# jackbaggins/RayTracing2-fork

Measured on AMD Instinct MI355X. Metric: Msamples/sec at 1920×1080 Cornell+OBJ; per-pixel RMSE vs CPU ref, higher is better.
Workload: dtype f32

## Files before the change

### raytracing2-fork_amd/csrc/device/rt2_k5_resident.h

```cpp
#pragma once

extern "C" __device__ int rt2_writelane(int value, int lane, int old) __asm("llvm.amdgcn.writelane.i32");

namespace {

constexpr int kResGroups = 38;

struct K5Resident {
    h8 rec[kResGroups * 4 * 64];
};

template <MfmaSpec S>
__device__ __forceinline__ bool exact_group(unsigned long long M, int G, int n_tris, cfloat* tri, const f3& o,
                                            const f3& d, float& best, int& bi, float& bestK, MfmaDiag& dg) {
    if constexpr (S.diag) dg.hot += 1;
    uint32_t m32 = (uint32_t)(M | M >> 32);
    const float bk0 = bestK;
    while (m32) {
        const int tt = __builtin_ctz(m32);
        m32 &= m32 - 1;
        const int idx = 32 * G + tt;
        if (idx >= n_tris) break;
        if constexpr (S.diag) dg.exact += 1;
        cfloat* tp = tri + 12 * idx;
        const MtQ qq = mt_quantities(o, d, ldc4(tp), ldc4(tp + 4), ldc4(tp + 8));
        if (mt_pass3(qq, bestK)) mt_exact(qq, idx, best, bi, bestK);
    }
    return __ballot(bestK != bk0) != 0;
}

__device__ __forceinline__ void xl_counts(MfmaDiag& dg, int pairs, int k, int rounds) {
    for (int off = 32; off > 0; off >>= 1) {
        pairs += __shfl_xor(pairs, off);
        k = max(k, __shfl_xor(k, off));
    }
    const unsigned long long kw = (unsigned long long)__builtin_amdgcn_readfirstlane(k);
    dg.xl[0] += (unsigned long long)__builtin_amdgcn_readfirstlane(pairs);
    dg.xl[1] += kw;
    dg.xl[2] += (unsigned long long)rounds;
    dg.xl[3] = kw > dg.xl[3] ? kw : dg.xl[3];
}

__host__ __device__ constexpr int xl_row_of_bit(int b) { return 8 * ((b & 15) >> 2) + 4 * (b >> 4) + (b & 3); }
__host__ __device__ constexpr int xl_bit_of_row(int r) { return 16 * ((r >> 2) & 1) + 4 * (r >> 3) + (r & 3); }

template <MfmaSpec S, bool YP, bool LDS, class Rebuild>
__device__ __forceinline__ void exact_window_lanes(int maskv, int Gw, bool more, int n_tris, const float4* tri4,
                                                   const h8* a0, const h8* y1, const h8* recs, bool upper, const f3& o,
                                                   const f3& d, float& best, int& bi, float& bestK, MfmaDiag& dg,
                                                   Rebuild rebuild, [[maybe_unused]] const int* slot_tri = nullptr) {
    const int lane = (int)lane_id();
    [[maybe_unused]] unsigned long long tc = 0;
    if constexpr (S.diag) {
        dg.claims += 1;
        tc = __builtin_amdgcn_s_memtime();
    }
    if (n_tris & 31) maskv = lane == (n_tris >> 5) - Gw ? maskv & (int)((1u << (n_tris & 31)) - 1u) : maskv;
    unsigned long long hotg = __ballot(maskv != 0);
    if constexpr (S.diag) dg.hot += (unsigned long long)__popcll(hotg);
    const float bk0 = bestK;
    const int src = 4 * xl_bit_of_row(lane & 31);
    const f16v zero = {};
    uint32_t m = 0;
    int gj = 0;
    [[maybe_unused]] int pairs = 0, iters = 0, rounds = 0;
#pragma nounroll
    for (;;) {
        int lst = 0, c = 0;
#pragma nounroll
        while (c < 32) {
            if (!m) {
                if (!hotg) break;
                gj = __builtin_ctzll(hotg);
                hotg &= hotg - 1;
                m = (uint32_t)__builtin_amdgcn_readlane(maskv, gj);
            }
            const int idx = 32 * (Gw + gj) + __builtin_ctz(m);
            m &= m - 1;
            lst = lane == c ? idx : lst;
            c++;
        }
        if (!c) break;
        if constexpr (S.diag) {
            dg.exact += (unsigned long long)c;
// ... 29 lines not shown
        };
        const int mk0 = block(0);
        int mk1 = 0;
        if (upper) mk1 = block(1);
        const auto sw = __builtin_amdgcn_permlane32_swap((uint32_t)mk0, (uint32_t)mk1, false, false);
        uint32_t pm = (sw[0] | sw[1] << 16) & (c == 32 ? ~0u : (1u << c) - 1u);
        if constexpr (S.diag) pairs += __popc(pm);
        auto entry = [&](uint32_t m) { return __builtin_amdgcn_ds_bpermute(4 * __builtin_ctz(m | 0x80000000u), lst); };
        struct Tri {
            int idx;
            float4 t0, t1, t2;
        };
        auto fetch = [&](Tri& t) {
            t.idx = entry(pm);
            t.t0 = tri4[3 * t.idx], t.t1 = tri4[3 * t.idx + 1], t.t2 = tri4[3 * t.idx + 2];
        };
        auto step = [&](const Tri& cur, Tri& nxt) {
            if constexpr (S.diag) iters += 1;
            const bool has = pm != 0;
            pm &= pm - 1;
            fetch(nxt);
            if (has) {
                const MtQ qq = mt_quantities(o, d, cur.t0, cur.t1, cur.t2);
                if (mt_pass3(qq, bestK)) {
                    if constexpr (S.slot_order)
                        mt_exact_slot(qq, cur.idx, slot_tri, best, bi, bestK);
                    else
                        mt_exact(qq, cur.idx, best, bi, bestK);
                }
            }
        };
        Tri ta, tb2;
        fetch(ta);
#pragma nounroll
        while (__ballot(pm != 0)) {
            step(ta, tb2);
            if (!__ballot(pm != 0)) break;
            step(tb2, ta);
        }
        if (c < 32) break;
    }
    if constexpr (S.diag) xl_counts(dg, pairs, iters, rounds);
    if (more && __ballot(bestK != bk0)) {
        if constexpr (S.diag) tc = __builtin_amdgcn_s_memtime();
        rebuild();
        if constexpr (S.diag) dg.t_pub += __builtin_amdgcn_s_memtime() - tc;
    }
}

template <MfmaSpec S, class Rebuild>
__device__ __forceinline__ void exact_window(uint32_t m1, int maskv, int Gw, int cnt, bool more, int n_tris,
                                             cfloat* tri, const f3& o, const f3& d, float& best, int& bi,
                                             float& bestK, MfmaDiag& dg, Rebuild rebuild) {
    constexpr int W = S.exact_win;
    auto mask_of = [&](int j) { return W == 1 ? m1 : (uint32_t)__builtin_amdgcn_readlane(maskv, j); };
    [[maybe_unused]] unsigned long long tc = 0;
    if constexpr (S.diag) {
        dg.claims += 1;
        tc = __builtin_amdgcn_s_memtime();
        int j = 0;
        while (!mask_of(j)) j++;
        const int idx = 32 * (Gw + j) + __builtin_ctz(mask_of(j));
        if (idx < n_tris) asm volatile("" ::"s"(__float_as_int(tri[12 * idx])));
        const unsigned long long t = __builtin_amdgcn_s_memtime();
        dg.t_issue += t - tc;
    }
    const float bk0 = bestK;
    [[maybe_unused]] int pairs = 0, tested = 0;
    for (int j = 0; j < cnt; j++) {
        uint32_t m32 = mask_of(j);
        if constexpr (S.diag) dg.hot += m32 != 0;
// ... 102 lines not shown
    const uint32_t dst = row + (row & 16);
    const auto sw = __builtin_amdgcn_permlane32_swap(dst, dst, false, false);
    const int half = (l & 32) >> 1;
    const int to0 = 4 * ((int)sw[0] + half), to1 = 4 * ((int)sw[1] + half);
    const u4 b0 = __builtin_bit_cast(u4, a0[0]), b1 = __builtin_bit_cast(u4, a0[1]);
    const bool first = (l & 15) < c0, keep = (l & 0x28) == 0;
    u4 r;
#pragma unroll
    for (int k = 0; k < 4; k++) {
        const int x0 = __builtin_amdgcn_ds_permute(to0, (int)b0[k]);
        const int x1 = __builtin_amdgcn_ds_permute(to1, (int)b1[k]);
        const uint32_t q = (uint32_t)(first ? x0 : x1);
        const uint32_t up = __builtin_amdgcn_permlane32_swap(0u, q, false, false)[0];
        const uint32_t sh = (uint32_t)__builtin_amdgcn_update_dpp(0, (int)up, 0x118, 0xf, 0xf, true);
        r[k] = keep ? q : sh;
    }
    return __builtin_bit_cast(h8, r);
}

struct SlotImage {
    const float4* tri4;
    const int* slot_tri;
};
__device__ __forceinline__ SlotImage slot_image(const RenderParams& p) {
    const int ng = (p.n_tris + 31) >> 5;
    const char* tab = reinterpret_cast<const char*>(reinterpret_cast<const h8*>(p.mfma_kt_frag) + (size_t)ng * (kKtOps * 64));
    const float4* t4 = reinterpret_cast<const float4*>(tab + sizeof(rt2_cluster_table));
    return {t4, reinterpret_cast<const int*>(t4 + 3 * (size_t)p.n_tris)};
}

template <MfmaSpec S>
__device__ __forceinline__ bool sweep_kt_res(const RenderParams& p, const h8* rec, const f3& o, const f3& d,
                                             float& best, int& bi, float& bestK, MfmaDiag& dg, bool upper,
                                             unsigned long long act = 0, ClusterDiag* cd = nullptr) {
    const int lane = (int)lane_id();
    [[maybe_unused]] unsigned long long tc = 0, tsw = 0;
    if constexpr (S.diag) tsw = tc = __builtin_amdgcn_s_memtime();
    auto stamp = [&](unsigned long long& acc) {
        if constexpr (S.diag) {
            const unsigned long long t = __builtin_amdgcn_s_memtime();
            acc += t - tc;
            tc = t;
        }
    };
    const f3 m = cross(d, o);
    MfmaScale sc;
    if (!mfma_scale<true>(p.mfma_A, o, d, m, sc)) return false;
    h8 a0[2], y1[2];
    _Float16 tw16;
    kt_frags<S.kt_lane_w>(d, m, sc, a0, tw16);
    constexpr bool per_group = S.exact_win == 1 && !S.y_skip_last && !S.diag;
    if constexpr (per_group || S.y_first) kt_y(d, o, bestK, sc, tw16, y1);
    stamp(dg.t_wait);
    const int ng = (p.n_tris + 31) >> 5, n_tris = p.n_tris;
    const int nres = S.res_l2 ? min(ng, kResGroups) : ng;
    cfloat* const tri = (cfloat*)p.tri;
    const h8* tb = rec + lane;
    [[maybe_unused]] const int* slot_tri = nullptr;
    if constexpr (S.slot_order) {
        static_assert(S.cluster_rows && S.exact_lanes && !S.res_l2, "slot_order: 353 / 354's one resident window");
        slot_tri = slot_image(p).slot_tri;
    }
    if constexpr (per_group) {
        for (int G = 0; G < nres; G++) {
            const h8 b0 = tb[0], b1 = tb[64], b2 = tb[128], b3 = tb[192];
            tb += kKtOps * 64;
            const unsigned long long M = kt_group(a0, y1, b0, b1, b2, b3, upper);
// ... 182 lines not shown
                            } else {
                                h8 af = a0[0];
                                if (upper) af = cluster_rows_frag(a0, need);
                                one_block(af, g0, g1);
                            }
                        }
                        maskv = lane < kNeedLane ? maskv : 0;
                    }
                }
            } else {
                for (int j = 0; j < cnt; j++) {
                    const h8 b0 = tb[0], b1 = tb[64], b2 = tb[128];
                    h8 b3 = {};
                    if constexpr (YP) b3 = tb[192];
                    tb += kKtOps * 64;
                    const unsigned long long M = kt_group<YP>(a0, y1, b0, b1, b2, b3, upper);
                    const uint32_t m32 = (uint32_t)(M | M >> 32);
                    if constexpr (W > 1) maskv = lane == j ? (int)m32 : maskv;
                    any |= m32;
                }
            }
            if constexpr (S.diag) dg.groups += (unsigned long long)cnt;
            if (resident) stamp(dg.t_filt);
            if (any) {
                const bool more = YP && (Gw + cnt < ng || (W == 1 && !S.y_skip_last));
                if (resident) phase_prio<S>(1);
                if constexpr (S.exact_lanes) {
                    static_assert(W > 1, "exact_lanes reads the window's masks from maskv");
                    const float4* tri4 = reinterpret_cast<const float4*>(p.tri);
                    if constexpr (S.slot_order) tri4 = slot_image(p).tri4;
                    auto rebuild = [&] { kt_y(d, o, bestK, sc, tw16, y1); };
                    if (!YP || resident)
                        exact_window_lanes<S, YP, true>(maskv, Gw, more, n_tris, tri4, a0, y1, rec, upper, o, d, best,
                                                        bi, bestK, dg, rebuild, slot_tri);
                    else if constexpr (YP)
                        exact_window_lanes<S, YP, false>(maskv, Gw, more, n_tris, tri4, a0, y1,
                                                         reinterpret_cast<const h8*>(p.mfma_kt_frag), upper, o, d, best,
                                                         bi, bestK, dg, rebuild);
                } else {
                    exact_window<S>(any, maskv, Gw, cnt, more, n_tris, tri, o, d, best, bi, bestK, dg,
                                    [&] { kt_y(d, o, bestK, sc, tw16, y1); });
                }
                if (resident) phase_prio<S>(0);
            }
            if constexpr (!YP && (S.res_l2 || W < kResGroups))
                if (Gw + cnt < ng) {
                    [[maybe_unused]] unsigned long long ty = 0;
                    if constexpr (S.diag) ty = __builtin_amdgcn_s_memtime();
                    kt_y(d, o, bestK, sc, tw16, y1);
                    if constexpr (S.diag) dg.t_pub += __builtin_amdgcn_s_memtime() - ty;
                }
            if (resident) stamp(dg.t_exact);
        };
        auto windows = [&](auto yfirst, const h8* tb, int G0, int G1, bool resident) {
            constexpr bool YF = decltype(yfirst)::value;
            int Gw = G0;
            if constexpr (!YF) {
                if (Gw < G1) window(std::false_type{}, tb, Gw, G1, resident);
                Gw += W;
            }
            if constexpr (YF || W < kResGroups)
                for (; Gw < G1; Gw += W) window(std::true_type{}, tb, Gw, G1, resident);
        };
        windows(std::bool_constant<S.y_first>{}, tb, 0, nres, true);
        if constexpr (S.res_l2)
            windows(std::true_type{}, reinterpret_cast<const h8*>(p.mfma_kt_frag) + (size_t)nres * (kKtOps * 64) + lane,
                    nres, ng, false);
// ... 16 lines not shown
        const h8* src = reinterpret_cast<const h8*>(p.mfma_kt_frag) + (size_t)pc * 64 + lane;
        __builtin_amdgcn_global_load_lds((const __attribute__((address_space(1))) void*)src,
                                         (__attribute__((address_space(3))) void*)&rs.rec[pc * 64], 16, 0, 0);
    }
    asm volatile("s_waitcnt vmcnt(0)" ::: "memory");
    __syncthreads();
}

template <MfmaSpec S>
__global__ __launch_bounds__(S.block) __attribute__((amdgpu_waves_per_eu(S.waves))) void render_mfma_k5r(RenderParams p_arg) {
    constexpr int NW = S.block / 64;
    __shared__ K5Resident rs;
    {
        const RenderParams& p = kargs<RenderParams>();
        const int ng = min((p.n_tris + 31) >> 5, kResGroups);
        const int lane = (int)lane_id(), wave = (int)(threadIdx.x >> 6);
        constexpr bool no_t1 = !S.y_first && S.exact_win >= kResGroups && !S.res_l2;
        for (int i = wave; i < (no_t1 ? 3 : 4) * ng; i += NW) {
            const int pc = no_t1 ? i + i / 3 : i;
            const h8* src = reinterpret_cast<const h8*>(p.mfma_kt_frag) + (size_t)pc * 64 + lane;
            __builtin_amdgcn_global_load_lds((const __attribute__((address_space(1))) void*)src,
                                             (__attribute__((address_space(3))) void*)&rs.rec[pc * 64], 16, 0, 0);
        }
        asm volatile("s_waitcnt vmcnt(0)" ::: "memory");
        __syncthreads();
    }
    Lane L;
    lane_init(L);
    MfmaDiag dg;
    struct NoClusterDiag {};
    [[maybe_unused]] std::conditional_t<S.cluster_rows8, ClusterDiag8,
                                        std::conditional_t<S.cluster_rows, ClusterDiag, NoClusterDiag>> cdg;
    [[maybe_unused]] PathDiagSlot<S.diag> pds;
    const int wave = (int)(threadIdx.x >> 6);
    [[maybe_unused]] unsigned long long segs_w = 0;
    [[maybe_unused]] unsigned long long wl_t0 = 0, wl_c0 = 0, wl_dry = 0, wl_r2 = 0, wl_r1 = 0, wl_coop = 0;
    if constexpr (S.diag) {
        wl_t0 = __builtin_amdgcn_s_memrealtime();
        wl_c0 = __builtin_amdgcn_s_memtime();
    }
    for (;;) {
        const RenderParams& p = kargs<RenderParams>();
        if constexpr (S.cam_park) {
            constexpr bool no_t1 = !S.y_first && S.exact_win >= kResGroups && !S.res_l2;
            static_assert(no_t1 && S.lean && NW <= kResGroups, "cam_park parks in T1 pieces that nothing else uses");
            float4* park = reinterpret_cast<float4*>(&rs.rec[(4 * wave + 3) * 64 + (int)lane_id()]);
            if constexpr (S.diag)
                advance<1, false, true, true, S.linear>(L, p, park, pds.get());
            else
                advance<1, false, true, false, S.linear>(L, p, park);
        } else if constexpr (S.diag) {
            advance<1, !S.lean, false, true, S.linear>(L, p, nullptr, pds.get());
        } else {
            advance<1, !S.lean, false, false, S.linear>(L, p);
        }
        unsigned long long act = __ballot(L.st == ST_TRACE);
        if constexpr (S.lean) segs_w += (unsigned long long)__popcll(act);
        if constexpr (S.diag) {
            if (!wl_dry && __any(L.st == ST_DONE)) wl_dry = __builtin_amdgcn_s_memrealtime();
            if (act) {
                if (__popcll(act) <= (unsigned)S.tail_lanes && __any(L.st == ST_DONE))
                    wl_coop++;
                else if (__popcll(act) <= 32)
                    wl_r1++;
                else
                    wl_r2++;
            }
// ... 26 lines not shown
                __builtin_amdgcn_s_setprio(0);
        }
        bool upper = true;
        if (__popcll(act) <= 32) {
            if (act >> 32) {
                const uint32_t l = lane_id(), nl = (uint32_t)__popcll(act);
                const bool live = (act >> l) & 1ull;
                const int to = 4 * (int)(live ? lanes_below(act) : nl + lanes_below(~act));
                lane_permute<!S.lean, !S.lean>(L, to);
                if constexpr (S.cam_park) {
                    float4* park = reinterpret_cast<float4*>(&rs.rec[(4 * wave + 3) * 64 + (int)lane_id()]);
                    const float4 e = *park;
                    *park = make_float4(perm_f(to, e.x), perm_f(to, e.y), perm_f(to, e.z), 0.0f);
                }
                act = __ballot(L.st == ST_TRACE);
            }
            upper = false;
        }
        const int j0 = __builtin_ctzll(act);
        const bool mine = L.st == ST_TRACE;
        {
            const f3 o = mk(__shfl(L.o.x, j0), __shfl(L.o.y, j0), __shfl(L.o.z, j0));
            const f3 dd = mk(__shfl(L.d.x, j0), __shfl(L.d.y, j0), __shfl(L.d.z, j0));
            if (!mine) {
                L.o = o;
                L.d = dd;
            }
        }
        const f3 ro = L.o, rd = L.d;
        float best = 1e38f, bestK = 1e38f * 1.0009765625f;
        int bi = -1;
        phase_prio<S>(0);
        bool swept;
        if constexpr (S.cluster_rows)
            swept = sweep_kt_res<S>(p, rs.rec, ro, rd, best, bi, bestK, dg, upper, act, &cdg);
        else
            swept = sweep_kt_res<S>(p, rs.rec, ro, rd, best, bi, bestK, dg, upper);
        if (!swept) coop_each(act, ro, rd, p, best, bi);
        phase_prio<S>(2);
        if (mine) {
            L.bounce += 1;
            if constexpr (!S.lean) L.segs += 1;
            if constexpr (S.diag)
                shade<1, true, S.linear>(L, p, best, bi, pds.get());
            else
                shade<1, false, S.linear>(L, p, best, bi);
        }
    }
    const RenderParams& p = kargs<RenderParams>();
    if constexpr (S.lean) {
        if (lane_id() == 0) atomicAdd(p.seg_counter, segs_w);
    } else {
        flush_counters(L, p);
    }
    if constexpr (S.diag)
        if (p.wave_log) {
            const uint32_t gw = blockIdx.x * NW + (uint32_t)wave;
            const unsigned long long c1 = __builtin_amdgcn_s_memtime();
            const unsigned long long hw = (unsigned long long)__builtin_amdgcn_s_getreg((31 << 11) | 4) |
                                          (unsigned long long)__builtin_amdgcn_s_getreg((15 << 11) | 20) << 32;
            if (lane_id() == 0 && gw < p.wave_log_n) {
                unsigned long long* e = p.wave_log + 10 * (size_t)gw;
                e[0] = wl_t0;
                e[1] = wl_dry;
                e[2] = __builtin_amdgcn_s_memrealtime();
                e[3] = wl_r2;
                e[4] = wl_r1;
// ... 12 lines not shown
        }
        if (lane_id() == 0) {
            atomicAdd(p.seg_counter + 20, calls);
            atomicAdd(p.seg_counter + 21, trips);
        }
    }
    if constexpr (S.diag)
        if (lane_id() == 0) {
            atomicAdd(p.seg_counter + 1, dg.groups);
            atomicAdd(p.seg_counter + 2, dg.hot);
            atomicAdd(p.seg_counter + 3, dg.exact);
            atomicAdd(p.seg_counter + 12, dg.t_wait);
            atomicAdd(p.seg_counter + 13, dg.t_filt);
            atomicAdd(p.seg_counter + 14, dg.t_exact);
            atomicAdd(p.seg_counter + 15, dg.t_swp);
            atomicAdd(p.seg_counter + 16, __builtin_amdgcn_s_memtime() - wl_c0);
            atomicAdd(p.seg_counter + 17, dg.t_issue);
            atomicAdd(p.seg_counter + 18, dg.t_pub);
            atomicAdd(p.seg_counter + 19, dg.claims);
            atomicAdd(p.seg_counter + 7, dg.xl[0]);
            atomicAdd(p.seg_counter + 8, dg.xl[1]);
            atomicAdd(p.seg_counter + 9, dg.xl[2]);
            atomicMax(p.seg_counter + 10, dg.xl[3]);
            atomicAdd(p.seg_counter + 22, pds.d.new_ray);
            atomicAdd(p.seg_counter + 23, pds.d.new_px);
            if constexpr (S.cluster_rows) {
                atomicAdd(p.seg_counter + 24, cdg.skipped);
                atomicAdd(p.seg_counter + 25, cdg.one);
                atomicAdd(p.seg_counter + 26, cdg.two);
                atomicAdd(p.seg_counter + 27, cdg.rays);
                atomicAdd(p.seg_counter + 28, cdg.r16);
                if constexpr (S.cluster_rows8) atomicAdd(p.seg_counter + 30, cdg.r8);
            }
        }
}

}
```

### raytracing2-fork_amd/csrc/device/rt2_mfma.h

```cpp
#pragma once

namespace {

typedef _Float16 h8 __attribute__((ext_vector_type(8)));
typedef float f4v __attribute__((ext_vector_type(4)));
typedef float f16v __attribute__((ext_vector_type(16)));

constexpr int kMfmaQ = 5;
constexpr float kMfmaC = 1.0009765625f;
constexpr float kMfmaTs = 0x1p-12f;
constexpr float kMfmaB = 2.0f;

struct MfmaSpec {
    int block;
    int waves;
    int tail_lanes;
    bool diag = false;
    int tile_groups = 0;
    bool fair_prio = false;
    int phase_prio = 0;
    bool flow_prio = false;
    bool kt_lane_w = false;
    bool lean = false;
    bool res_l2 = false;
    int exact_win = 1;
    bool y_skip_last = false;
    bool y_first = false;
    bool exact_lanes = false;
    bool pair_loop = false;
    bool cam_park = false;
    bool cluster_rows = false;
    bool cluster_rows16 = false;
    bool cluster_rows8 = false;
    bool slot_order = false;
    bool linear = false;
};

struct MfmaDiag {
    unsigned long long groups = 0, hot = 0, exact = 0;
    unsigned long long xl[4] = {};
    unsigned long long t_wait = 0, t_filt = 0, t_exact = 0, t_swp = 0;
    unsigned long long unused1 = 0;
    unsigned long long t_issue = 0, t_pub = 0, claims = 0;
};

struct MfmaCoef {
    double c[kMfmaQ][10];
    double tau;
};
__device__ __forceinline__ void mfma_coefs(const float4* tri, int i, int n, MfmaCoef& k, uint32_t* flags) {
    for (int q = 0; q < kMfmaQ; q++)
        for (int c = 0; c < 10; c++) k.c[q][c] = 0.0;
    k.tau = 1.0;
    if (i >= n) {
        k.c[3][9] = 0x1p13;
        return;
    }
    const float4 t0 = tri[3 * i], t1 = tri[3 * i + 1], t2 = tri[3 * i + 2];
    const float a[3] = {t0.x, t0.y, t0.z}, e0[3] = {t0.w, t1.x, t1.y}, e1[3] = {t1.z, t1.w, t2.x},
                nn[3] = {t2.y, t2.z, t2.w};
    bool ok = true;
    float A = 0.0f, M = 0.0f;
    for (int j = 0; j < 3; j++) {
        ok = ok && fabsf(a[j]) <= 0x1p20f;
        A = fmaxf(A, fabsf(a[j]));
        for (float x : {e0[j], e1[j], nn[j]}) {
            const float ax = fabsf(x);
            ok = ok && (x == 0.0f || (ax >= 0x1p-100f && ax <= 0x1p20f));
// ... 1001 lines not shown
```

### raytracing2-fork_amd/csrc/device/rt2_render.hip

```cpp
#include <hip/hip_runtime.h>

#include <algorithm>
#include <cstdio>
#include <cstdlib>
#include <cstring>
#include <mutex>
#include <numeric>
#include <string>
#include <type_traits>
#include <vector>

#include "../../../include/rt2.h"
#include "../../../include/rt2_cluster.h"
#include "rt2_math.h"

using namespace rt2d;

#include "rt2_sweep.h"
#include "rt2_path.h"
#include "rt2_brute.h"
#include "rt2_mfma.h"
#include "rt2_k5_tiles.h"
#include "rt2_k5_resident.h"
#include "rt2_assist.h"
// ... 557 lines not shown
    x.y_first = true;
    return x;
}
#endif
constexpr MfmaSpec kt_xl(MfmaSpec x) {
    x.exact_lanes = true;
    return x;
}
constexpr MfmaSpec kt_pair(MfmaSpec x) {
    x.pair_loop = true;
    return x;
}
constexpr MfmaSpec kt_park(MfmaSpec x) {
    x.cam_park = true;
    return x;
}
constexpr MfmaSpec kt_cr(MfmaSpec x) {
    x.cluster_rows = true;
    return x;
}
constexpr MfmaSpec kt_cr16(MfmaSpec x) {
    x.cluster_rows = true;
    x.cluster_rows16 = true;
    return x;
}
constexpr MfmaSpec kt_cr8(MfmaSpec x) {
    x.cluster_rows8 = true;
    return x;
}
constexpr MfmaSpec kt_slot(MfmaSpec x) {
    x.slot_order = true;
    return x;
}
constexpr int kResWin = 38;
constexpr int kResL2Groups = 256;
constexpr MfmaSpec kt_tiles_flow() {
    return MfmaSpec{.block = 768, .waves = 3, .tail_lanes = 0, .tile_groups = 19, .flow_prio = true, .kt_lane_w = true};
}
constexpr MfmaSpec kt_tiles_flow4() {
    MfmaSpec x = kt_tiles_flow();
    x.block = 1024;
    x.waves = 4;
    x.lean = true;
    return x;
}
constexpr MfmaSpec kResFrame = kt_win(kt_res(false, false, true, 4), kResWin);
constexpr MfmaSpec kResSlabFrame = kt_win(kt_res(false, true, true), kResWin);
constexpr MfmaSpec kt_product(MfmaSpec frame) { return kt_slot(kt_cr8(kt_cr16(kt_park(kt_pair(kt_xl(frame)))))); }
constexpr MfmaSpec kRes = kt_product(kResFrame);
constexpr MfmaSpec kResSlab = kt_product(kResSlabFrame);
constexpr MfmaSpec kResL2 = kt_win(kt_res(true, false, true, 4), kResWin);
constexpr MfmaSpec kResL2Slab = kt_win(kt_res(true, true, true), kResWin);
constexpr MfmaSpec kTiles = kt_tiles_flow4();
constexpr Bvh3Spec kBvhDefault{.block = 256, .thresh = 16, .slab = Slab::Markstein, .waves = 5, .diag = false};

#ifdef RT2_EXPERIMENTS
constexpr SmemSpec smem_x(int g, Filter f, Tail t, int lanes, int w, bool stats = false) {
    return SmemSpec{.block = 256, .group = g, .filter = f, .tail = t, .tail_lanes = lanes, .waves = w, .stats = stats};
}
constexpr SplitSpec split_x(int s, Filter f, int w) {
    return SplitSpec{.waves_per_ray = s, .group = 8, .filter = f, .waves = w};
}
constexpr Bvh3Spec bvh3_x(int t, Slab sl, int w, bool diag = false) {
    return Bvh3Spec{.block = 256, .thresh = t, .slab = sl, .waves = w, .diag = diag};
}
#endif

constexpr Variant kVariants[] = {
    RT2_VARIANT(0, K_SMEM, render_smem<kSmemDefault>, 256, "smem/256/max3f8/coop32/w6/lockstep"),
    RT2_PRODUCT(109, K_BVH4, render_bvh4, kBvhDefault, 256, "bvh4/256/t16/w5"),
    RT2_PRODUCT(86, K_TILED, render_tiled, kTiledLarge, 512, "tiled/512/max3f4"),
    RT2_PRODUCT(92, K_ASSIST, render_assist, kAssist12, 768, "assist12/max3f8/w6"),
    RT2_PRODUCT(136, K_SMEM, render_smem, kSmemDefault, 256, "smem/256/max3f8/coop32/w6/lockstep"),
    RT2_PRODUCT(227, K_MFMA, render_mfma, kMfmaK5, 256, "mfma/256/k5/coop8/w3/imax/minred/ymma/t12/llds/ser4/cmp"),
    RT2_PRODUCT(353, K_MFMA, render_mfma_k5r, kRes, 1024, "mfmar/1024/kt4/res38/coop4/w4/cmp/dpp/lean/lw/pp4", kResGroups, true),
    RT2_PRODUCT(354, K_MFMA, render_mfma_k5r, kResSlab, 1024, "mfmar/1024/kt4/res38/coop4/w4/cmp/fair/dpp/lean/lw", kResGroups, true),
    RT2_PRODUCT(355, K_MFMA, render_mfma_k5r, kResL2, 1024, "mfmarl2/1024/kt4/res38l2/coop4/w4/cmp/dpp/lean/lw/pp4", kResL2Groups),
    RT2_PRODUCT(356, K_MFMA, render_mfma_k5r, kResL2Slab, 1024, "mfmarl2/1024/kt4/res38l2/coop4/w4/cmp/fair/dpp/lean/lw", kResL2Groups),
    RT2_PRODUCT(380, K_MFMA, render_mfma_k5t, kTiles, 1024, "mfmat5/1024/kt4/tile19/coop0/w4/cmp/regs/perm/lw/flowp/lean"),
#ifdef RT2_EXPERIMENTS
    RT2_VARIANT(342, K_MFMA, render_mfma_k5r<kt_win(kt_res(false, false, false), kResWin)>, 1024, "mfmar/1024/kt4/res38/coop4/w4/cmp/dpp/lean", kResGroups),
// ... 7 lines not shown
    RT2_VARIANT(350, K_MFMA, render_mfma_k5r<kt_win(kt_res(false, false, true, 0, true), kResWin)>, 1024, "mfmar/1024/kt4/res38/coop4/w4/cmp/diag/dpp/lean/lw", kResGroups),
    RT2_VARIANT(390, K_MFMA, render_mfma_k5r<kt_win(kt_res(false, false, true, 0, true), 1)>, 1024, "mfmar/1024/kt4/res38/coop4/w4/cmp/diag/dpp/lean/lw/xw1", kResGroups),
    RT2_VARIANT(392, K_MFMA, render_mfma_k5r<kt_win(kt_res(false, false, true, 4), 1)>, 1024, "mfmar/1024/kt4/res38/coop4/w4/cmp/dpp/lean/lw/pp4/xw1", kResGroups),
    RT2_VARIANT(393, K_MFMA, render_mfma_k5r<kt_win(kt_res(false, false, true, 4), 1, true)>, 1024, "mfmar/1024/kt4/res38/coop4/w4/cmp/dpp/lean/lw/pp4/xw1s", kResGroups),
    RT2_VARIANT(394, K_MFMA, render_mfma_k5r<kt_win(kt_res(false, false, true, 4), 2)>, 1024, "mfmar/1024/kt4/res38/coop4/w4/cmp/dpp/lean/lw/pp4/xw2", kResGroups),
    RT2_VARIANT(395, K_MFMA, render_mfma_k5r<kt_win(kt_res(false, false, true, 4), 4)>, 1024, "mfmar/1024/kt4/res38/coop4/w4/cmp/dpp/lean/lw/pp4/xw4", kResGroups),
    RT2_VARIANT(396, K_MFMA, render_mfma_k5r<kt_win(kt_res(false, false, true, 4), 8)>, 1024, "mfmar/1024/kt4/res38/coop4/w4/cmp/dpp/lean/lw/pp4/xw8", kResGroups),
    RT2_VARIANT(399, K_MFMA, render_mfma_k5r<kt_win(kt_res(false, false, true, 4), 19)>, 1024, "mfmar/1024/kt4/res38/coop4/w4/cmp/dpp/lean/lw/pp4/xw19", kResGroups),
    RT2_VARIANT(397, K_MFMA, render_mfma_k5r<kt_win(kt_res(true, false, true, 4), 1)>, 1024, "mfmarl2/1024/kt4/res38l2/coop4/w4/cmp/dpp/lean/lw/pp4/xw1", kResL2Groups),
    RT2_VARIANT(398, K_MFMA, render_mfma_k5r<kt_win(kt_res(false, true, true), 1)>, 1024, "mfmar/1024/kt4/res38/coop4/w4/cmp/fair/dpp/lean/lw/xw1", kResGroups),
    RT2_VARIANT(351, K_MFMA, render_mfma_k5r<kt_yw(kt_win(kt_res(false, false, true, 4), kResWin))>, 1024, "mfmar/1024/kt4/res38/coop4/w4/cmp/dpp/lean/lw/pp4/yw", kResGroups),
    RT2_VARIANT(352, K_MFMA, render_mfma_k5r<kt_yw(kt_win(kt_res(true, false, true, 4), kResWin))>, 1024, "mfmarl2/1024/kt4/res38l2/coop4/w4/cmp/dpp/lean/lw/pp4/yw", kResL2Groups),
    RT2_VARIANT(357, K_MFMA, render_mfma_k5r<kt_yw(kt_win(kt_res(false, false, true, 0, true), kResWin))>, 1024, "mfmar/1024/kt4/res38/coop4/w4/cmp/diag/dpp/lean/lw/yw", kResGroups),
    RT2_VARIANT(400, K_MFMA, render_mfma_k5r<kt_win(kt_res(false, false, true, 4), kResWin)>, 1024, "mfmar/1024/kt4/res38/coop4/w4/cmp/dpp/lean/lw/pp4/xwave", kResGroups),
    RT2_VARIANT(401, K_MFMA, render_mfma_k5r<kt_xl(kt_win(kt_res(true, false, true, 4), kResWin))>, 1024, "mfmarl2/1024/kt4/res38l2/coop4/w4/cmp/dpp/lean/lw/pp4/xl", kResL2Groups),
    RT2_VARIANT(402, K_MFMA, render_mfma_k5r<kt_xl(kt_win(kt_res(false, false, true, 0, true), kResWin))>, 1024, "mfmar/1024/kt4/res38/coop4/w4/cmp/diag/dpp/lean/lw/xl", kResGroups),
    RT2_VARIANT(403, K_MFMA, render_mfma_k5r<kt_win(kt_res(false, true, true), kResWin)>, 1024, "mfmar/1024/kt4/res38/coop4/w4/cmp/fair/dpp/lean/lw/xwave", kResGroups),
    RT2_VARIANT(404, K_MFMA, render_mfma_k5r<kt_xl(kt_win(kt_res(true, true, true), kResWin))>, 1024, "mfmarl2/1024/kt4/res38l2/coop4/w4/cmp/fair/dpp/lean/lw/xl", kResL2Groups),
    RT2_VARIANT(405, K_MFMA, render_mfma_k5r<kt_xl(kt_win(kt_res(false, false, true, 4), kResWin))>, 1024, "mfmar/1024/kt4/res38/coop4/w4/cmp/dpp/lean/lw/pp4/nopair/nopark", kResGroups),
    RT2_VARIANT(406, K_MFMA, render_mfma_k5r<kt_pair(kt_xl(kt_win(kt_res(false, false, true, 4), kResWin)))>, 1024, "mfmar/1024/kt4/res38/coop4/w4/cmp/dpp/lean/lw/pp4/nopark", kResGroups),
    RT2_VARIANT(407, K_MFMA, render_mfma_k5r<kt_park(kt_xl(kt_win(kt_res(false, false, true, 4), kResWin)))>, 1024, "mfmar/1024/kt4/res38/coop4/w4/cmp/dpp/lean/lw/pp4/nopair", kResGroups),
    RT2_VARIANT(408, K_MFMA, render_mfma_k5r<kt_xl(kt_win(kt_res(false, true, true), kResWin))>, 1024, "mfmar/1024/kt4/res38/coop4/w4/cmp/fair/dpp/lean/lw/nopair/nopark", kResGroups),
    RT2_VARIANT(409, K_MFMA, render_mfma_k5r<kt_park(kt_pair(kt_xl(kt_win(kt_res(false, false, true, 4), kResWin))))>, 1024, "mfmar/1024/kt4/res38/coop4/w4/cmp/dpp/lean/lw/pp4/nocr", kResGroups),
    RT2_VARIANT(410, K_MFMA, render_mfma_k5r<kt_park(kt_pair(kt_xl(kt_win(kt_res(false, true, true), kResWin))))>, 1024, "mfmar/1024/kt4/res38/coop4/w4/cmp/fair/dpp/lean/lw/nocr", kResGroups),
    RT2_VARIANT(411, K_MFMA, render_mfma_k5r<kt_cr16(kt_pair(kt_xl(kt_win(kt_res(false, false, true, 0, true), kResWin))))>, 1024, "mfmar/1024/kt4/res38/coop4/w4/cmp/diag/dpp/lean/lw/xl/cr16", kResGroups),
    RT2_VARIANT(412, K_MFMA, render_mfma_k5r<kt_cr(kt_park(kt_pair(kt_xl(kt_win(kt_res(false, false, true, 4), kResWin)))))>, 1024, "mfmar/1024/kt4/res38/coop4/w4/cmp/dpp/lean/lw/pp4/cr32", kResGroups),
    RT2_VARIANT(413, K_MFMA, render_mfma_k5r<kt_cr(kt_park(kt_pair(kt_xl(kt_win(kt_res(false, true, true), kResWin)))))>, 1024, "mfmar/1024/kt4/res38/coop4/w4/cmp/fair/dpp/lean/lw/cr32", kResGroups),
    RT2_VARIANT(414, K_MFMA, render_mfma_k5r<kt_cr16(kt_park(kt_pair(kt_xl(kt_win(kt_res(false, false, true, 4), kResWin)))))>, 1024, "mfmar/1024/kt4/res38/coop4/w4/cmp/dpp/lean/lw/pp4/idx", kResGroups),
    RT2_VARIANT(415, K_MFMA, render_mfma_k5r<kt_cr16(kt_park(kt_pair(kt_xl(kt_win(kt_res(false, true, true), kResWin)))))>, 1024, "mfmar/1024/kt4/res38/coop4/w4/cmp/fair/dpp/lean/lw/idx", kResGroups),
    RT2_VARIANT(416, K_MFMA, render_mfma_k5r<kt_slot(kt_cr16(kt_pair(kt_xl(kt_win(kt_res(false, false, true, 0, true), kResWin)))))>, 1024, "mfmar/1024/kt4/res38/coop4/w4/cmp/diag/dpp/lean/lw/xl/cr16/slot", kResGroups, true),
    RT2_VARIANT(417, K_MFMA, render_mfma_k5r<kt_slot(kt_cr16(kt_park(kt_pair(kt_xl(kt_win(kt_res(false, false, true, 4), kResWin))))))>, 1024, "mfmar/1024/kt4/res38/coop4/w4/cmp/dpp/lean/lw/pp4/r16", kResGroups, true),
    RT2_VARIANT(418, K_MFMA, render_mfma_k5r<kt_slot(kt_cr16(kt_park(kt_pair(kt_xl(kt_win(kt_res(false, true, true), kResWin))))))>, 1024, "mfmar/1024/kt4/res38/coop4/w4/cmp/fair/dpp/lean/lw/r16", kResGroups, true),
    RT2_VARIANT(419, K_MFMA, render_mfma_k5r<kt_slot(kt_cr8(kt_cr16(kt_pair(kt_xl(kt_win(kt_res(false, false, true, 0, true), kResWin))))))>, 1024, "mfmar/1024/kt4/res38/coop4/w4/cmp/diag/dpp/lean/lw/xl/cr8/slot", kResGroups, true),
    RT2_VARIANT(370, K_MFMA, render_mfma_k5t<kt_tiles_flow()>, 768, "mfmat5/768/kt4/tile19/coop0/w3/cmp/regs/perm/lw/flowp"),
    RT2_VARIANT(368, K_MFMA, render_mfma_k5t<[] { MfmaSpec x = kt_tiles_flow(); x.diag = true; return x; }()>, 768, "mfmat5/768/kt4/tile19/coop0/w3/cmp/regs/perm/lw/flowp/diag"),
    RT2_VARIANT(369, K_MFMA, render_mfma_k5t<[] { MfmaSpec x = kt_tiles_flow(); x.flow_prio = false; return x; }()>, 768, "mfmat5/768/kt4/tile19/coop0/w3/cmp/regs/perm/lw/flow"),
    RT2_VARIANT(382, K_MFMA, render_mfma_k5t<[] { MfmaSpec x = kt_tiles_flow(); x.lean = true; return x; }()>, 768, "mfmat5/768/kt4/tile19/coop0/w3/cmp/regs/perm/lw/flowp/lean"),
    RT2_VARIANT(381, K_MFMA, render_mfma_k5t<[] { MfmaSpec x = kt_tiles_flow4(); x.tile_groups = 16; return x; }()>, 1024, "mfmat5/1024/kt4/tile16/coop0/w4/cmp/regs/perm/lw/flowp/lean"),
    RT2_VARIANT(385, K_MFMA, render_mfma_k5t<[] { MfmaSpec x = kt_tiles_flow4(); x.flow_prio = false; return x; }()>, 1024, "mfmat5/1024/kt4/tile19/coop0/w4/cmp/regs/perm/lw/flow/lean"),
    RT2_VARIANT(386, K_MFMA, render_mfma_k5t<[] { MfmaSpec x = kt_tiles_flow4(); x.tail_lanes = 4; return x; }()>, 1024, "mfmat5/1024/kt4/tile19/coop4/w4/cmp/regs/perm/lw/flowp/lean"),
    RT2_VARIANT(67, K_SMEM, render_smem<kSmemMid>, 256, "smem/256/max3f8/coop32"),
    RT2_VARIANT(85, K_SPLIT, render_split<kSplitSmall>, 256, "split4/max3f8/w6"),
    RT2_VARIANT(53, K_BVH3, render_bvh3<kBvhDefault>, 256, "bvh3/256/t16/w5"),
    RT2_VARIANT(106, K_SMEM, render_smem<kSmemFree>, 256, "smem/256/max3f8/coop32/w6/free"),
    RT2_VARIANT(37, K_BVH, render_bvh<BvhSpec{256}>, 256, "bvh/256"),
    RT2_VARIANT(40, K_BVH2, (render_bvh2<Bvh2Spec{256, 16}>), 256, "bvh2/256/t16"),
    RT2_VARIANT(41, K_BVH2, (render_bvh2<Bvh2Spec{256, 8}>), 256, "bvh2/256/t8"),
    RT2_VARIANT(43, K_BVH2, (render_bvh2<Bvh2Spec{128, 16}>), 128, "bvh2/128/t16"),
    RT2_VARIANT(45, K_BVH2, (render_bvh2<Bvh2Spec{256, 1}>), 256, "bvh2/256/t1"),
    RT2_VARIANT(46, K_BVH3, render_bvh3<bvh3_x(16, Slab::Markstein, 1)>, 256, "bvh3/256/t16"),
    RT2_VARIANT(47, K_BVH3, render_bvh3<bvh3_x(8, Slab::Markstein, 1)>, 256, "bvh3/256/t8"),
    RT2_VARIANT(48, K_BVH3, render_bvh3<bvh3_x(24, Slab::Markstein, 1)>, 256, "bvh3/256/t24"),
    RT2_VARIANT(50, K_BVH3, render_bvh3<bvh3_x(16, Slab::Binary64, 1)>, 256, "bvh3/256/t16/div64"),
    RT2_VARIANT(54, K_BVH3, render_bvh3<bvh3_x(8, Slab::Markstein, 5)>, 256, "bvh3/256/t8/w5"),
    RT2_VARIANT(55, K_BVH3, render_bvh3<bvh3_x(16, Slab::Filtered, 5)>, 256, "bvh3/256/t16/filt/w5"),
    RT2_VARIANT(58, K_BVH3, render_bvh3<bvh3_x(16, Slab::Markstein, 5, true)>, 256, "bvh3/256/t16/w5/DIAG"),
    RT2_VARIANT(64, K_SMEM, render_smem<smem_x(8, Filter::Five, Tail::Team, 32, 1)>, 256, "smem/256/masked8/team32"),
    RT2_VARIANT(66, K_SMEM, render_smem<smem_x(8, Filter::Five, Tail::Team, 64, 1)>, 256, "smem/256/masked8/team64"),
    RT2_VARIANT(74, K_SMEM, render_smem<smem_x(4, Filter::Plk, Tail::Coop, 32, 1)>, 256, "smem/256/plk4/coop32"),
    RT2_VARIANT(76, K_SMEM, render_smem<smem_x(8, Filter::Plk, Tail::Coop, 32, 1)>, 256, "smem/256/plk8/coop32"),
    RT2_VARIANT(79, K_SMEM, render_smem<smem_x(8, Filter::Plk, Tail::Coop, 32, 6)>, 256, "smem/256/plk8/coop32/w6"),
    RT2_VARIANT(80, K_SMEM, render_smem<smem_x(2, Filter::Plk, Tail::Coop, 32, 1)>, 256, "smem/256/plk2/coop32"),
    RT2_VARIANT(82, K_SMEM, render_smem<smem_x(8, Filter::Max3, Tail::Coop, 32, 1, true)>, 256,
                "smem/256/max3f8/coop32/STATS"),
#endif
};
// ... 1225 lines not shown
```

Measured before the change: 2011.

## Spread leftover exact triangle tests across idle lanes via LDS work list

After each lane handles its first candidate triangle in the exact window, the remaining (lane, triangle) pairs are prefix-summed with a DPP scan and written to an LDS list. When they fit in one wave pass, each lane takes one pair, pulls that ray's origin, direction and best hit with ds_bpermute, and runs the exact Möller–Trumbore test. Results merge back through a wave-scoped 64-bit atomic min per ray slot. This replaces the divergent serial loop over remaining hits, at the cost of LDS traffic, permutes and atomics, and it becomes the default in kt_product.

```diff
diff --git a/raytracing2-fork_amd/csrc/device/rt2_k5_resident.h b/raytracing2-fork_amd/csrc/device/rt2_k5_resident.h
--- a/raytracing2-fork_amd/csrc/device/rt2_k5_resident.h
+++ b/raytracing2-fork_amd/csrc/device/rt2_k5_resident.h
@@ -44,12 +44,37 @@
 __host__ __device__ constexpr int xl_row_of_bit(int b) { return 8 * ((b & 15) >> 2) + 4 * (b >> 4) + (b & 3); }
 __host__ __device__ constexpr int xl_bit_of_row(int r) { return 16 * ((r >> 2) & 1) + 4 * (r >> 3) + (r & 3); }
 
+template <int CTRL, int ROW_MASK>
+__device__ __forceinline__ int dpp_add_step(int x) {
+    return x + __builtin_amdgcn_update_dpp(0, x, CTRL, ROW_MASK, 0xf, false);
+}
+__device__ __forceinline__ int exact_spread_scan(int r, int& at) {
+    int x = r;
+    x = dpp_add_step<0x111, 0xf>(x);
+    x = dpp_add_step<0x112, 0xf>(x);
+    x = dpp_add_step<0x114, 0xf>(x);
+    x = dpp_add_step<0x118, 0xf>(x);
+    x = dpp_add_step<0x142, 0xa>(x);
+    x = dpp_add_step<0x143, 0xc>(x);
+    at = x - r;
+    return __builtin_amdgcn_readlane(x, 63);
+}
+
 template <MfmaSpec S, bool YP, bool LDS, class Rebuild>
 __device__ __forceinline__ void exact_window_lanes(int maskv, int Gw, bool more, int n_tris, const float4* tri4,
                                                    const h8* a0, const h8* y1, const h8* recs, bool upper, const f3& o,
                                                    const f3& d, float& best, int& bi, float& bestK, MfmaDiag& dg,
-                                                   Rebuild rebuild, [[maybe_unused]] const int* slot_tri = nullptr) {
+                                                   Rebuild rebuild, [[maybe_unused]] const int* slot_tri = nullptr,
+                                                   [[maybe_unused]] unsigned long long* xs_diag = nullptr,
+                                                   [[maybe_unused]] int xs_wave = 0) {
     const int lane = (int)lane_id();
+    [[maybe_unused]] uint32_t* xs_list = nullptr;
+    [[maybe_unused]] unsigned long long* xs_slot = nullptr;
+    constexpr bool XS = S.exact_spread && LDS && !YP;
+    if constexpr (XS) {
+        xs_list = reinterpret_cast<uint32_t*>(const_cast<h8*>(recs) + (4 * (16 + xs_wave) + 3) * 64);
+        xs_slot = reinterpret_cast<unsigned long long*>(xs_list + 128);
+    }
     [[maybe_unused]] unsigned long long tc = 0;
     if constexpr (S.diag) {
         dg.claims += 1;
@@ -145,11 +170,95 @@
         };
         Tri ta, tb2;
         fetch(ta);
+        if constexpr (XS) {
+            {
+                if constexpr (S.diag) iters += 1;
+                const bool has = pm != 0;
+                pm &= pm - 1;
+                if (has) {
+                    const MtQ qq = mt_quantities(o, d, ta.t0, ta.t1, ta.t2);
+                    if (mt_pass3(qq, bestK)) {
+                        if constexpr (S.slot_order)
+                            mt_exact_slot(qq, ta.idx, slot_tri, best, bi, bestK);
+                        else
+                            mt_exact(qq, ta.idx, best, bi, bestK);
+                    }
+                }
+            }
+            const int r = __popc(pm);
+            int at;
+            const int Rw = exact_spread_scan(r, at);
+            if (Rw) {
+                const bool spread = Rw <= 64 && __ballot(r >= 2) != 0;
+                if constexpr (S.diag) {
+                    xs_diag[0] += (unsigned long long)Rw;
+                    xs_diag[1] += spread ? 1ull : Rw > 64 ? 1ull << 40 : 0ull;
+                }
+                if (spread) {
+                    int wl = lane;
+                    asm volatile("" : "+v"(wl));
+                    xs_slot[wl] = ~0ull;
+                    while (pm) {
+                        xs_list[at++] = (uint32_t)lane | (uint32_t)__builtin_ctz(pm) << 8;
+                        pm &= pm - 1;
+                    }
+                    asm volatile("" ::: "memory");
+                    const bool work = lane < Rw - (S.spread_drop ? 1 : 0);
+                    const uint32_t e = work ? xs_list[wl] : 0u;
+                    const int from = 4 * (int)(e & 63u);
+                    Tri tw;
+                    tw.idx = __builtin_amdgcn_ds_bpermute(4 * (int)(e >> 8 & 31u), lst);
+                    tw.t0 = tri4[3 * tw.idx], tw.t1 = tri4[3 * tw.idx + 1], tw.t2 = tri4[3 * tw.idx + 2];
+                    int wtri = tw.idx;
+                    if constexpr (S.slot_order) wtri = slot_tri[tw.idx];
+                    auto pull = [&](float v) {
+                        return __int_as_float(__builtin_amdgcn_ds_bpermute(from, __float_as_int(v)));
+                    };
+                    const f3 so = mk(pull(o.x), pull(o.y), pull(o.z));
+                    const f3 sd = mk(pull(d.x), pull(d.y), pull(d.z));
+                    float cbest = pull(best);
+                    int cbi = __builtin_amdgcn_ds_bpermute(from, bi);
+                    float cbestK = cbest * 1.0009765625f;
+                    if (work) {
+                        const MtQ qq = mt_quantities(so, sd, tw.t0, tw.t1, tw.t2);
+                        if (mt_pass3(qq, cbestK)) {
+                            if constexpr (S.slot_order)
+                                mt_exact_slot(qq, tw.idx, slot_tri, cbest, cbi, cbestK);
+                            else
+                                mt_exact(qq, tw.idx, cbest, cbi, cbestK);
+                            if (cbi == tw.idx) {
+                                const uint32_t lo = S.slot_order ? (uint32_t)wtri << 16 | (uint32_t)tw.idx
+                                                                 : (uint32_t)tw.idx;
+                                __hip_atomic_fetch_min(&xs_slot[e & 63u],
+                                                       (unsigned long long)__float_as_uint(cbest) << 32 | lo,
+                                                       __ATOMIC_RELAXED, __HIP_MEMORY_SCOPE_WAVEFRONT);
+                            }
+                        }
+                    }
+                    asm volatile("" ::: "memory");
+                    const unsigned long long key = xs_slot[wl];
+                    if (key != ~0ull) {
+                        best = __uint_as_float((uint32_t)(key >> 32));
+                        bi = (int)((uint32_t)key & (S.slot_order ? 0xffffu : ~0u));
+                        bestK = best * 1.0009765625f;
+                    }
+                } else {
+                    fetch(ta);
 #pragma nounroll
-        while (__ballot(pm != 0)) {
-            step(ta, tb2);
-            if (!__ballot(pm != 0)) break;
-            step(tb2, ta);
+                    while (__ballot(pm != 0)) {
+                        step(ta, tb2);
+                        if (!__ballot(pm != 0)) break;
+                        step(tb2, ta);
+                    }
+                }
+            }
+        } else {
+#pragma nounroll
+            while (__ballot(pm != 0)) {
+                step(ta, tb2);
+                if (!__ballot(pm != 0)) break;
+                step(tb2, ta);
+            }
         }
         if (c < 32) break;
     }
@@ -318,7 +427,9 @@
 template <MfmaSpec S>
 __device__ __forceinline__ bool sweep_kt_res(const RenderParams& p, const h8* rec, const f3& o, const f3& d,
                                              float& best, int& bi, float& bestK, MfmaDiag& dg, bool upper,
-                                             unsigned long long act = 0, ClusterDiag* cd = nullptr) {
+                                             unsigned long long act = 0, ClusterDiag* cd = nullptr,
+                                             [[maybe_unused]] unsigned long long* xs_diag = nullptr,
+                                             [[maybe_unused]] int xs_wave = 0) {
     const int lane = (int)lane_id();
     [[maybe_unused]] unsigned long long tc = 0, tsw = 0;
     if constexpr (S.diag) tsw = tc = __builtin_amdgcn_s_memtime();
@@ -567,7 +678,7 @@
                     auto rebuild = [&] { kt_y(d, o, bestK, sc, tw16, y1); };
                     if (!YP || resident)
                         exact_window_lanes<S, YP, true>(maskv, Gw, more, n_tris, tri4, a0, y1, rec, upper, o, d, best,
-                                                        bi, bestK, dg, rebuild, slot_tri);
+                                                        bi, bestK, dg, rebuild, slot_tri, xs_diag, xs_wave);
                     else if constexpr (YP)
                         exact_window_lanes<S, YP, false>(maskv, Gw, more, n_tris, tri4, a0, y1,
                                                          reinterpret_cast<const h8*>(p.mfma_kt_frag), upper, o, d, best,
@@ -650,7 +761,18 @@
     [[maybe_unused]] std::conditional_t<S.cluster_rows8, ClusterDiag8,
                                         std::conditional_t<S.cluster_rows, ClusterDiag, NoClusterDiag>> cdg;
     [[maybe_unused]] PathDiagSlot<S.diag> pds;
+    struct SpreadDiag {
+        unsigned long long n[2] = {};
+    };
+    [[maybe_unused]] std::conditional_t<S.exact_spread && S.diag, SpreadDiag, NoClusterDiag> xsd;
+    if constexpr (S.exact_spread) {
+        constexpr bool no_t1 = !S.y_first && S.exact_win >= kResGroups && !S.res_l2;
+        static_assert(no_t1 && NW <= 16 && 2 * NW <= kResGroups && S.exact_lanes,
+                      "exact_spread works in T1 pieces that nothing else uses");
+    }
     const int wave = (int)(threadIdx.x >> 6);
+    [[maybe_unused]] int xs_wave = 0;
+    if constexpr (S.exact_spread) xs_wave = __builtin_amdgcn_readfirstlane(wave);
     [[maybe_unused]] unsigned long long segs_w = 0;
     [[maybe_unused]] unsigned long long wl_t0 = 0, wl_c0 = 0, wl_dry = 0, wl_r2 = 0, wl_r1 = 0, wl_coop = 0;
     if constexpr (S.diag) {
@@ -743,7 +865,11 @@
         int bi = -1;
         phase_prio<S>(0);
         bool swept;
-        if constexpr (S.cluster_rows)
+        if constexpr (S.exact_spread && S.diag)
+            swept = sweep_kt_res<S>(p, rs.rec, ro, rd, best, bi, bestK, dg, upper, act, &cdg, xsd.n, xs_wave);
+        else if constexpr (S.exact_spread)
+            swept = sweep_kt_res<S>(p, rs.rec, ro, rd, best, bi, bestK, dg, upper, act, &cdg, nullptr, xs_wave);
+        else if constexpr (S.cluster_rows)
             swept = sweep_kt_res<S>(p, rs.rec, ro, rd, best, bi, bestK, dg, upper, act, &cdg);
         else
             swept = sweep_kt_res<S>(p, rs.rec, ro, rd, best, bi, bestK, dg, upper);
@@ -822,7 +948,11 @@
                 atomicAdd(p.seg_counter + 28, cdg.r16);
                 if constexpr (S.cluster_rows8) atomicAdd(p.seg_counter + 30, cdg.r8);
             }
-        }
-}
-
-}
+            if constexpr (S.exact_spread) {
+                atomicAdd(p.seg_counter + 4, xsd.n[0]);
+                atomicAdd(p.seg_counter + 11, xsd.n[1]);
+            }
+        }
+}
+
+}
diff --git a/raytracing2-fork_amd/csrc/device/rt2_mfma.h b/raytracing2-fork_amd/csrc/device/rt2_mfma.h
--- a/raytracing2-fork_amd/csrc/device/rt2_mfma.h
+++ b/raytracing2-fork_amd/csrc/device/rt2_mfma.h
@@ -34,6 +34,8 @@
     bool cluster_rows8 = false;
     bool slot_order = false;
     bool linear = false;
+    bool exact_spread = false;
+    bool spread_drop = false;
 };
 
 struct MfmaDiag {
diff --git a/raytracing2-fork_amd/csrc/device/rt2_render.hip b/raytracing2-fork_amd/csrc/device/rt2_render.hip
--- a/raytracing2-fork_amd/csrc/device/rt2_render.hip
+++ b/raytracing2-fork_amd/csrc/device/rt2_render.hip
@@ -613,6 +613,10 @@
     x.slot_order = true;
     return x;
 }
+constexpr MfmaSpec kt_spread(MfmaSpec x) {
+    x.exact_spread = true;
+    return x;
+}
 constexpr int kResWin = 38;
 constexpr int kResL2Groups = 256;
 constexpr MfmaSpec kt_tiles_flow() {
@@ -627,7 +631,9 @@
 }
 constexpr MfmaSpec kResFrame = kt_win(kt_res(false, false, true, 4), kResWin);
 constexpr MfmaSpec kResSlabFrame = kt_win(kt_res(false, true, true), kResWin);
-constexpr MfmaSpec kt_product(MfmaSpec frame) { return kt_slot(kt_cr8(kt_cr16(kt_park(kt_pair(kt_xl(frame)))))); }
+constexpr MfmaSpec kt_product(MfmaSpec frame) {
+    return kt_spread(kt_slot(kt_cr8(kt_cr16(kt_park(kt_pair(kt_xl(frame)))))));
+}
 constexpr MfmaSpec kRes = kt_product(kResFrame);
 constexpr MfmaSpec kResSlab = kt_product(kResSlabFrame);
 constexpr MfmaSpec kResL2 = kt_win(kt_res(true, false, true, 4), kResWin);
@@ -701,6 +707,10 @@
     RT2_VARIANT(417, K_MFMA, render_mfma_k5r<kt_slot(kt_cr16(kt_park(kt_pair(kt_xl(kt_win(kt_res(false, false, true, 4), kResWin))))))>, 1024, "mfmar/1024/kt4/res38/coop4/w4/cmp/dpp/lean/lw/pp4/r16", kResGroups, true),
     RT2_VARIANT(418, K_MFMA, render_mfma_k5r<kt_slot(kt_cr16(kt_park(kt_pair(kt_xl(kt_win(kt_res(false, true, true), kResWin))))))>, 1024, "mfmar/1024/kt4/res38/coop4/w4/cmp/fair/dpp/lean/lw/r16", kResGroups, true),
     RT2_VARIANT(419, K_MFMA, render_mfma_k5r<kt_slot(kt_cr8(kt_cr16(kt_pair(kt_xl(kt_win(kt_res(false, false, true, 0, true), kResWin))))))>, 1024, "mfmar/1024/kt4/res38/coop4/w4/cmp/diag/dpp/lean/lw/xl/cr8/slot", kResGroups, true),
+    RT2_VARIANT(420, K_MFMA, render_mfma_k5r<kt_slot(kt_cr8(kt_cr16(kt_park(kt_pair(kt_xl(kResFrame))))))>, 1024, "mfmar/1024/kt4/res38/coop4/w4/cmp/dpp/lean/lw/pp4/loop", kResGroups, true),
+    RT2_VARIANT(421, K_MFMA, render_mfma_k5r<kt_slot(kt_cr8(kt_cr16(kt_park(kt_pair(kt_xl(kResSlabFrame))))))>, 1024, "mfmar/1024/kt4/res38/coop4/w4/cmp/fair/dpp/lean/lw/loop", kResGroups, true),
+    RT2_VARIANT(422, K_MFMA, render_mfma_k5r<kt_spread(kt_slot(kt_cr8(kt_cr16(kt_pair(kt_xl(kt_win(kt_res(false, false, true, 0, true), kResWin)))))))>, 1024, "mfmar/1024/kt4/res38/coop4/w4/cmp/diag/dpp/lean/lw/xl/cr8/slot/spread", kResGroups, true),
+    RT2_VARIANT(423, K_MFMA, render_mfma_k5r<[] { MfmaSpec x = kRes; x.spread_drop = true; return x; }()>, 1024, "mfmar/1024/kt4/res38/coop4/w4/cmp/dpp/lean/lw/pp4/drop", kResGroups, true),
     RT2_VARIANT(370, K_MFMA, render_mfma_k5t<kt_tiles_flow()>, 768, "mfmat5/768/kt4/tile19/coop0/w3/cmp/regs/perm/lw/flowp"),
     RT2_VARIANT(368, K_MFMA, render_mfma_k5t<[] { MfmaSpec x = kt_tiles_flow(); x.diag = true; return x; }()>, 768, "mfmat5/768/kt4/tile19/coop0/w3/cmp/regs/perm/lw/flowp/diag"),
     RT2_VARIANT(369, K_MFMA, render_mfma_k5t<[] { MfmaSpec x = kt_tiles_flow(); x.flow_prio = false; return x; }()>, 768, "mfmat5/768/kt4/tile19/coop0/w3/cmp/regs/perm/lw/flow"),
```

Measured after the change: 2063, median of 6. 1.03x the previous value.
